# UBC-ECE-Sasha/PIM-compression

Measured on AMD Instinct MI355X. Metric: end-to-end GB/s (compress + decompress) on Silesia-mix; bit-exact ratio parity, higher is better.
Workload: dtype u8; 1 GPU; silesia_mix 8 x 1024 MiB containers in all (BASELINE configs[4]), block_size 32768; containers_this_rank=8, container_bytes=1073741824, block_size=32768, parallelism=whole containers dealt over 1 GPU(s), no collective

## Files before the change

### pim-compression_amd/csrc/snappy_k1_stream.hpp

```cpp
#pragma once

namespace snappy_hip {


#ifdef SNAPPY_PROF
__device__ unsigned long long g_prof[32];
struct StreamProf {
    unsigned long long acc = 0, cnt = 0, last = 0;
};
#define PROF_START() (prof.last = __builtin_readcyclecounter())
#define PROF_LAP(i) do { const unsigned long long now_ = __builtin_readcyclecounter(); if (lane == (i)) { prof.acc += now_ - prof.last; prof.cnt++; } prof.last = now_; } while (0)
#define PROF_WAIT() __builtin_amdgcn_s_waitcnt(0)
#define PROF_FLUSH() do { if (lane < 16) { atomicAdd(&g_prof[lane], prof.acc); atomicAdd(&g_prof[16 + lane], prof.cnt); } } while (0)
#elif defined(SNAPPY_MARK)
struct StreamProf {};
#define PROF_START() asm volatile("; PHASE start")
#define PROF_LAP(i) asm volatile("; PHASE " #i)
#define PROF_WAIT() ((void)0)
#define PROF_FLUSH() ((void)0)
#else
struct StreamProf {};
#define PROF_START() ((void)0)
#define PROF_LAP(i) ((void)0)
#define PROF_WAIT() ((void)0)
#define PROF_FLUSH() ((void)0)
#endif

template <class T, class = void> struct table_gathers_once : std::false_type {};
template <class T> struct table_gathers_once<T, std::void_t<decltype(T::kGathersOnce)>> : std::true_type {};

constexpr uint32_t kStreamRoom = 192;
#ifndef SNAPPY_STREAM_SLOTS_LDS
#define SNAPPY_STREAM_SLOTS_LDS 512
#endif
constexpr uint32_t kStreamSlotsLds = SNAPPY_STREAM_SLOTS_LDS, kStreamSlotsGlobal = 256;
__host__ __device__ constexpr uint32_t stream_scratch_bytes(uint32_t slots) { return 8u * slots; }

struct StreamWindow {
    uint32_t base;
    uint4 a, b;
    uint32_t h0, e0;
};

__device__ __forceinline__ void stream_load_window(StreamWindow& w, const uint8_t* __restrict__ blk, uint32_t base, uint32_t last16,
                                                   uint32_t lane)
{
    w.base = base;
    const uint32_t q = base + lane;
    w.a = ld128(blk + (q < last16 ? q : last16));
    w.b = ld128(blk + (q + 16u < last16 ? q + 16u : last16));
}
__device__ __forceinline__ void stream_hash_window(StreamWindow& w, uint32_t shift)
{
    const uint32_t prod = w.a.x * kHashMul;
    w.h0 = prod >> shift;
    w.e0 = (prod << (32 - shift)) & 0xffff0000u;
}

struct StreamGather {
    uint32_t ent;
    uint4 ka, kb;
    unsigned long long worthm;
};
template <class Table>
__device__ __forceinline__ void stream_issue_gather(StreamGather& g, const Table& table, const StreamWindow& w,
                                                    const uint8_t* __restrict__ blk, uint32_t lane)
{
    const uint32_t mine_l = w.e0 | (w.base + lane);
    g.ent = table.load_lane(w.h0, mine_l);
    const bool worth = !Table::certain_miss(g.ent, mine_l);
    g.worthm = __ballot(worth);
    g.ka = g.kb = make_uint4(0, 0, 0, 0);
    if (worth) {
        const uint8_t* __restrict__ c = blk + (g.ent & 0xffffu);
        g.ka = ld128(c);
        g.kb = ld128(c + 16);
    }
}

#ifdef SNAPPY_EMU
__device__ __forceinline__ uint32_t lds_max_rtn(lds_words_t p, uint32_t v)
{
    const uint32_t old = *p;
    if (v > old) *p = v;
    return old;
}
#else
__device__ __forceinline__ uint32_t lds_max_rtn(lds_words_t p, uint32_t v)
{
    return __hip_atomic_fetch_max((__attribute__((address_space(3))) uint32_t*)p, v, __ATOMIC_RELAXED, __HIP_MEMORY_SCOPE_WAVEFRONT);
}
#endif

struct StreamDup {
    uint32_t j1 = 0;
    uint32_t extj = 0;
    unsigned long long nf = 0;
    unsigned long long hitj = 0;
    unsigned long long deep = 0;
    unsigned long long cx = 0;
};

template <uint32_t kSlots>
__device__ __forceinline__ void stream_analyse(StreamDup& d, const StreamWindow& w, lds_bytes_t scratch, uint32_t lane)
{
    lds_words_t tab = (lds_words_t)scratch;
    const uint32_t sa = w.h0 & (kSlots - 1u);
    const uint32_t sb = kSlots + ((w.h0 >> 5) & (kSlots - 1u));
#ifdef SNAPPY_EMU
    static const bool unordered = getenv("EMU_LDS_UNORDERED") != nullptr;
    uint32_t oa = 0, ob = 0;
    if (unordered) {
        oa = lds_max_rtn(tab + sa, lane + 1u);
        ob = lds_max_rtn(tab + sb, lane + 1u);
    } else {
        for (uint32_t turn = 0; turn < kWave; ++turn) {
            if (lane == turn) {
                oa = lds_max_rtn(tab + sa, lane + 1u);
                ob = lds_max_rtn(tab + sb, lane + 1u);
            }
            __builtin_amdgcn_wave_barrier();
        }
    }
#else
    const uint32_t oa = lds_max_rtn(tab + sa, lane + 1u);
    const uint32_t ob = lds_max_rtn(tab + sb, lane + 1u);
#endif
    __builtin_amdgcn_wave_barrier();
    tab[sa] = 0;
    tab[sb] = 0;
    __builtin_amdgcn_wave_barrier();
    const uint32_t ja = oa - 1u, jb = ob - 1u;
    d = StreamDup();
    if (__ballot((oa && ja >= lane) || (ob && jb >= lane))) {
        STREAM_STAT(7);
        ALIAS_STAT(3);
        d.cx = dup_slot_lanes(scratch, w.h0, lane);
        for (uint32_t i = lane; i < 2u * kSlots; i += kWave) tab[i] = 0;
        __builtin_amdgcn_wave_barrier();
        return;
    }
    const uint32_t ha = (uint32_t)__shfl((int)w.h0, (int)(ja & 63u));
    const uint32_t hb = (uint32_t)__shfl((int)w.h0, (int)(jb & 63u));
    const unsigned long long OA = __ballot(oa != 0), OB = __ballot(ob != 0);
    const unsigned long long MA = OA & __ballot(ha == w.h0), MB = OB & __ballot(hb == w.h0);
    const bool ma = __builtin_amdgcn_inverse_ballot_w64(MA);
    d.j1 = ma ? ja : jb;
    d.nf = MA | MB;
    d.cx = OA & OB & ~d.nf;
    for (unsigned long long m = d.cx; m; m &= m - 1) {
        const uint32_t s = (uint32_t)__builtin_ctzll(m);
        const uint32_t hs = (uint32_t)__builtin_amdgcn_readlane((int)w.h0, (int)s);
        ALIAS_STAT(0);
        if (__ballot(w.h0 == hs) & ((1ull << s) - 1ull)) {
            ALIAS_STAT(2);
        } else {
            ALIAS_STAT(1);
            d.cx &= ~(1ull << s);
        }
    }
    if (d.nf) {
        const uint32_t jl = d.j1 & 63u;
        const uint32_t xj = (uint32_t)__shfl((int)w.a.x, (int)jl);
        const uint32_t e1 = (uint32_t)__shfl((int)w.a.y, (int)jl) ^ w.a.y;
        const uint32_t e2 = (uint32_t)__shfl((int)w.a.z, (int)jl) ^ w.a.z;
        d.hitj = d.nf & __ballot(xj == w.a.x);
        d.extj = min_u32(min_u32(first_bit(e1), first_bit(e2) | 32u), 64u) >> 3;
        const unsigned long long chained = d.nf | d.cx;
        d.deep = d.nf & __ballot(((uint32_t)(chained >> jl) & 1u) != 0);
    }
}

__device__ __forceinline__ void stream_walk(uint32_t advv, uint32_t clv, uint32_t& t, unsigned long long& V, unsigned long long& COV)
{
#ifdef SNAPPY_EMU
    for (;;) {
        const uint32_t l = t & 63u;
        V |= 1ull << l;
        const uint32_t a = (uint32_t)__builtin_amdgcn_readlane((int)advv, (int)l);
        const uint32_t c = (uint32_t)__builtin_amdgcn_readlane((int)clv, (int)l);
        if (c) COV |= ((1ull << c) - 1ull) << l;
        const uint32_t nt = t + a;
        const bool carry = nt < t;
        t = nt;
        if (carry) break;
    }
#else
    uint32_t a, c;
    unsigned long long m;
    asm volatile(
        "1:\n"
        "  s_bitset1_b64 %[V], %[t]\n"
        "  v_readlane_b32 %[a], %[advv], %[t]\n"
        "  v_readlane_b32 %[c], %[clv], %[t]\n"
        "  s_bfm_b64 %[m], %[c], %[t]\n"
        "  s_or_b64 %[COV], %[COV], %[m]\n"
        "  s_add_u32 %[t], %[t], %[a]\n"
        "  s_cbranch_scc1 2f\n"
        "  s_bitset1_b64 %[V], %[t]\n"
        "  v_readlane_b32 %[a], %[advv], %[t]\n"
        "  v_readlane_b32 %[c], %[clv], %[t]\n"
        "  s_bfm_b64 %[m], %[c], %[t]\n"
        "  s_or_b64 %[COV], %[COV], %[m]\n"
        "  s_add_u32 %[t], %[t], %[a]\n"
        "  s_cbranch_scc1 2f\n"
        "  s_bitset1_b64 %[V], %[t]\n"
        "  v_readlane_b32 %[a], %[advv], %[t]\n"
        "  v_readlane_b32 %[c], %[clv], %[t]\n"
        "  s_bfm_b64 %[m], %[c], %[t]\n"
        "  s_or_b64 %[COV], %[COV], %[m]\n"
        "  s_add_u32 %[t], %[t], %[a]\n"
        "  s_cbranch_scc1 2f\n"
        "  s_bitset1_b64 %[V], %[t]\n"
        "  v_readlane_b32 %[a], %[advv], %[t]\n"
        "  v_readlane_b32 %[c], %[clv], %[t]\n"
        "  s_bfm_b64 %[m], %[c], %[t]\n"
        "  s_or_b64 %[COV], %[COV], %[m]\n"
        "  s_add_u32 %[t], %[t], %[a]\n"
        "  s_cbranch_scc0 1b\n"
        "2:\n"
        : [t] "+s"(t), [V] "+s"(V), [COV] "+s"(COV), [a] "=&s"(a), [c] "=&s"(c), [m] "=&s"(m)
        : [advv] "v"(advv), [clv] "v"(clv)
        : "scc");
#endif
}

#ifndef SNAPPY_EMU
__device__ __forceinline__ unsigned long long uni64(unsigned long long v)
{
    return (unsigned long long)uni((uint32_t)v) | ((unsigned long long)uni((uint32_t)(v >> 32)) << 32);
}
#else
__device__ __forceinline__ unsigned long long uni64(unsigned long long v) { return v; }
#endif

__device__ __forceinline__ uint32_t stream_past(uint32_t dist, unsigned long long inter, uint32_t land)
{
    if (land >= kWave || ((inter >> land) & 1ull)) return 0;
    return (uint32_t)__builtin_amdgcn_readlane((int)dist, (int)land);
}

__device__ __forceinline__ bool has_run_of_34(unsigned long long m)
{
    unsigned long long r = m & (m >> 1);
    r &= r >> 2;
    r &= r >> 4;
    r &= r >> 8;
    r &= r >> 16;
    return (r & (m >> 32) & (m >> 33)) != 0;
}

template <class Table>
__device__ __forceinline__ void stream_put(const Table& table, uint32_t x, uint32_t pos, uint32_t shift, uint32_t lane)
{
    const uint32_t prod = x * kHashMul;
    if constexpr (Table::kCollectiveStore)
        table.store_masked(1ull, prod >> shift, pos, lane);
    else
        table.put(prod >> shift, ((prod << (32 - shift)) & 0xffff0000u) | pos, lane);
}
template <class Table>
__device__ __forceinline__ void stream_store(const Table& table, const StreamWindow& w, unsigned long long m, uint32_t lane)
{
    if constexpr (Table::kCollectiveStore) {
        table.store_masked(m, w.h0, w.base + lane, lane);
    } else {
        if (__builtin_amdgcn_inverse_ballot_w64(m)) table.store_lane(w.h0, w.e0 | (w.base + lane));
        __builtin_amdgcn_wave_barrier();
    }
}

__device__ __forceinline__ void stream_emit(uint8_t* __restrict__ dst, const uint8_t* __restrict__ blk, uint32_t& op, uint32_t& next_emit,
                                            uint32_t base, uint32_t x0, uint32_t ent, uint32_t extv, unsigned long long H,
                                            unsigned long long COV, bool by_copy, uint32_t r_out, bool long_copy, uint32_t ip,
                                            uint32_t long_cand, uint32_t long_len, uint32_t lane)
{
    if (H) emit_segment<false>(dst, blk, op, next_emit, base, x0, ent, extv, H, COV, by_copy, r_out, lane);
    if (long_copy) {
        if (ip > next_emit) op = emit_literal_windowed<false>(dst, op, blk, next_emit, ip - next_emit, base, x0, lane);
        op = emit_copy(dst, op, ip - long_cand, long_len, lane);
        next_emit = ip + long_len;
    }
}

struct SoloMate {
    static constexpr bool kAnalysesInPlace = true;
    __device__ __forceinline__ void begin(uint32_t, uint32_t, uint32_t) {}
    __device__ __forceinline__ void drain(uint32_t&, uint32_t&, uint32_t) {}
    template <uint32_t kSlots>
    __device__ __forceinline__ void analysis(StreamDup& d, const StreamWindow& w, lds_bytes_t scratch, uint32_t lane)
    {
        stream_analyse<kSlots>(d, w, scratch, lane);
    }
    __device__ __forceinline__ void emit(uint8_t* __restrict__ dst, const uint8_t* __restrict__ blk, uint32_t& op, uint32_t& next_emit,
                                         uint32_t base, uint32_t x0, uint32_t ent, uint32_t extv, unsigned long long H,
                                         unsigned long long COV, bool by_copy, uint32_t r_out, bool long_copy, uint32_t ip,
                                         uint32_t long_cand, uint32_t long_len, uint32_t lane)
    {
        stream_emit(dst, blk, op, next_emit, base, x0, ent, extv, H, COV, by_copy, r_out, long_copy, ip, long_cand, long_len, lane);
    }
};

template <class Table, uint32_t kSlots, class Mate>
__device__ __forceinline__ void stream_run(const uint8_t* __restrict__ blk, uint32_t avail, uint32_t n, uint32_t shift,
                                           uint8_t* __restrict__ dst, const Table table, uint32_t lane, lds_bytes_t dup_scratch,
                                           ParseState& ps, StreamProf& prof, Mate& mate)
{
    const uint32_t limit = n - kInputMargin;
    const uint32_t last16 = avail - 16u;
    uint32_t ip = ps.ip, skip = ps.skip, op = ps.op, next_emit = ps.next_emit;
    mate.begin(op, next_emit, lane);

    for (;;) {
        StreamWindow cur, nxt;
        stream_load_window(cur, blk, ip & ~63u, last16, lane);
        stream_hash_window(cur, shift);
        StreamGather g;
        stream_issue_gather(g, table, cur, blk, lane);
        __builtin_amdgcn_sched_barrier(0);
        stream_load_window(nxt, blk, cur.base + 64u, last16, lane);
        StreamDup dup;
        mate.template analysis<kSlots>(dup, cur, dup_scratch, lane);
        PROF_LAP(0);
        bool restart = false;

        for (;;) {
            const uint32_t r0 = ip - cur.base;
            const uint32_t b_in = 64u - skip;
            PROF_WAIT();
            PROF_LAP(1);

            unsigned long long hitm = __ballot(g.ka.x == cur.a.x) & g.worthm;
            const uint32_t t1 = min_u32(first_bit(g.ka.y ^ cur.a.y), first_bit(g.ka.z ^ cur.a.z) | 32u);
            const uint32_t t2 = min_u32(first_bit(g.ka.w ^ cur.a.w), first_bit(g.kb.x ^ cur.b.x) | 32u) | 64u;
            const uint32_t t3 = min_u32(first_bit(g.kb.y ^ cur.b.y), first_bit(g.kb.z ^ cur.b.z) | 32u) | 128u;
            uint32_t extv = min_u32(min_u32(t1, t2), min_u32(t3, 192u)) >> 3;
            uint32_t ent = g.ent & 0xffffu;
            const unsigned long long pend = dup.nf & __ballot(dup.j1 >= r0);
            const unsigned long long satm = hitm & __ballot(extv == 24u);
            unsigned long long stopm = pend | dup.cx | satm;
            const unsigned long long above_r0 = ~0ull << r0;
            const unsigned long long inter = hitm | stopm;
            const unsigned long long up = (lane < 63u) ? (inter >> (lane + 1u)) : 0ull;
            const uint32_t dist = up ? (uint32_t)__builtin_ctzll(up) + 1u : 64u - lane;
            const bool stopl = __builtin_amdgcn_inverse_ballot_w64(stopm);
            const bool hitl = __builtin_amdgcn_inverse_ballot_w64(hitm);
            const uint32_t clt = hitl ? 4u + extv : 0u;
            const bool hitjl = __builtin_amdgcn_inverse_ballot_w64(dup.hitj);
            const uint32_t clj = hitjl ? 4u + dup.extj : 0u;
            const uint32_t land_t = lane + clt, land_j = lane + clj;
            const uint32_t dist_t = (uint32_t)__shfl((int)dist, (int)(land_t & 63u));
            const uint32_t dist_j = (uint32_t)__shfl((int)dist, (int)(land_j & 63u));
            const bool plain_t = land_t < 64u && !((inter >> (land_t & 63u)) & 1ull);
            const bool plain_j = land_j < 64u && !((inter >> (land_j & 63u)) & 1ull);
            const uint32_t advt = hitl ? clt + (plain_t ? dist_t : 0u) : dist;
            const uint32_t advj = hitjl ? clj + (plain_j ? dist_j : 0u) : dist;
            const unsigned long long satjm = dup.hitj & __ballot(dup.extj == 8u);
            uint32_t clv = stopl ? 0u : clt;
            uint32_t advv = stopl ? 64u : advt;
            PROF_LAP(2);

            unsigned long long V = 0, COV = 0;
            uint32_t t = r0 - 64u;
            uint32_t r_out = 0;
            bool long_copy = false;
            uint32_t long_cand = 0, long_len = 0;
            for (;;) {
                t = uni(t);
                stream_walk(advv, clv, t, V, COV);
                const uint32_t s = 63u - (uint32_t)__builtin_clzll(V);
                if (!((stopm >> s) & 1ull)) {
                    r_out = t + 64u;
                    break;
                }
                PROF_LAP(3);
                STREAM_STAT(3);
                const unsigned long long bit_s = 1ull << s;
                const unsigned long long below_s = bit_s - 1ull;
                const unsigned long long interior_s = COV & ~(V & hitm & below_s);
                uint32_t how = 0;
                uint32_t j = 0;
                if (pend & bit_s) {
                    j = (uint32_t)__builtin_amdgcn_readlane((int)dup.j1, (int)s);
                    const unsigned long long not_inserted = interior_s & (interior_s >> 1);
                    if (!((not_inserted >> j) & 1ull)) how = 1;
                    else if (dup.deep & bit_s) how = 2;
                }
                if (dup.cx & bit_s) how = 2;
#ifdef SNAPPY_EMU
                if (dup.cx & bit_s) ALIAS_STAT(4);
                else if (!(pend & bit_s)) ALIAS_STAT(8);
                else if (how == 2) ALIAS_STAT(5);
                else if (how == 1) ALIAS_STAT(7);
                else ALIAS_STAT(6);
#endif
                uint32_t adv_s, cl_s, cand_s = 0, sat_s = 24;
                bool hit_s, more_s;
                if (how == 2) {
                    STREAM_STAT(6);
                    const unsigned long long ins = ((above_r0 & below_s & ~interior_s) | (COV & ~(interior_s >> 1))) & below_s;
                    const uint32_t hs = (uint32_t)__builtin_amdgcn_readlane((int)cur.h0, (int)s);
                    const unsigned long long J = __ballot(cur.h0 == hs) & ins;
                    how = 0;
                    if (!J) ALIAS_STAT(9);
                    if (J) {
                        j = 63u - (uint32_t)__builtin_clzll(J);
                        hit_s = (uint32_t)__builtin_amdgcn_readlane((int)cur.a.x, (int)s) == (uint32_t)__builtin_amdgcn_readlane((int)cur.a.x, (int)j);
                        const uint32_t e1 = (uint32_t)__builtin_amdgcn_readlane((int)cur.a.y, (int)s) ^ (uint32_t)__builtin_amdgcn_readlane((int)cur.a.y, (int)j);
                        const uint32_t e2 = (uint32_t)__builtin_amdgcn_readlane((int)cur.a.z, (int)s) ^ (uint32_t)__builtin_amdgcn_readlane((int)cur.a.z, (int)j);
                        const uint32_t ext_s = e1 ? ((uint32_t)__builtin_ctz(e1) >> 3) : (e2 ? 4u + ((uint32_t)__builtin_ctz(e2) >> 3) : 8u);
                        cand_s = cur.base + j;
                        sat_s = 8;
                        more_s = hit_s && ext_s == 8u;
                        cl_s = hit_s ? 4u + ext_s : 0u;
                        adv_s = hit_s ? cl_s : (uint32_t)__builtin_amdgcn_readlane((int)dist, (int)s);
                        if (hit_s && !more_s) adv_s += stream_past(dist, hitm | stopm, s + cl_s);
                        how = 3;
                    }
                }
                if (how == 1) {
                    STREAM_STAT(9);
                    hit_s = (dup.hitj & bit_s) != 0;
                    more_s = (satjm & bit_s) != 0;
                    adv_s = (uint32_t)__builtin_amdgcn_readlane((int)advj, (int)s);
                    cl_s = (uint32_t)__builtin_amdgcn_readlane((int)clj, (int)s);
                    cand_s = cur.base + j;
                    sat_s = 8;
                } else if (how == 0) {
                    STREAM_STAT(10);
                    hit_s = (hitm & bit_s) != 0;
                    more_s = (satm & bit_s) != 0;
                    adv_s = (uint32_t)__builtin_amdgcn_readlane((int)advt, (int)s);
                    cl_s = (uint32_t)__builtin_amdgcn_readlane((int)clt, (int)s);
                }
                if (more_s) {
                    STREAM_STAT(8);
                    if (how == 0) cand_s = (uint32_t)__builtin_amdgcn_readlane((int)ent, (int)s);
                    cl_s = 4u + sat_s + match_extend(blk, cand_s + 4u + sat_s, cur.base + s + 4u + sat_s, n, lane);
                    adv_s = cl_s <= 63u ? cl_s + stream_past(dist, hitm | stopm, s + cl_s) : cl_s;
                    if (cl_s > 63u) {
                        STREAM_STAT(2);
                        V &= ~bit_s;
                        r_out = s;
                        long_copy = true;
                        long_cand = cand_s;
                        long_len = cl_s;
                        break;
                    }
                }
                stopm &= ~bit_s;
                hitm = hit_s ? (hitm | bit_s) : (hitm & ~bit_s);
                if (lane == s) {
                    advv = adv_s;
                    clv = cl_s;
                    if (how != 0) ent = cand_s;
                    if (how != 0 || more_s) extv = cl_s - 4u;
                }
                t = s - 64u;
                PROF_LAP(4);
            }
            PROF_LAP(3);

            const uint32_t r_end = r_out < kWave ? r_out : kWave;
            const unsigned long long range = r_end > r0 ? (above_r0 & lanes_below(r_end)) : 0ull;
            const unsigned long long H = V & hitm & range;
            const unsigned long long interior = COV & ~H;
            const unsigned long long probed = range & ~interior;
            const unsigned long long miss = probed & ~H;
            const uint32_t top = probed ? 63u - (uint32_t)__builtin_clzll(probed) : 0u;
            const bool by_copy = probed && ((H >> top) & 1ull);
            uint32_t skip_out = skip;
            bool widened = false;
            if (probed) {
                const uint32_t tail = by_copy ? 0u : (uint32_t)__builtin_clzll(~(miss << (63u - top)));
                const bool copy_before = (H & ((1ull << top) - 1ull)) != 0;
                const uint32_t allowed = copy_before ? 33u : b_in;
                if ((uint32_t)__builtin_popcountll(miss) > b_in) {
                    const uint32_t lead = (uint32_t)__builtin_ctzll(~(miss >> r0));
                    widened = lead > b_in || has_run_of_34(miss) || tail > allowed;
                }
                skip_out = by_copy ? 31u : 64u - (allowed - tail);
            }
            if (widened) {
                STREAM_STAT(1);
                break;
            }
            STREAM_STAT(0);

            unsigned long long endl = COV & ~(interior >> 1) & range;
            if (by_copy && r_out > kWave) endl &= ~(1ull << 63);
            unsigned long long C = probed | endl;
            if (long_copy) C |= 1ull << r_out;
            {
                const unsigned long long later = dup.nf | dup.cx;
                stream_store(table, cur, C & ~later, lane);
                const unsigned long long second = C & dup.nf & ~dup.deep & ~dup.cx;
                if (second) stream_store(table, cur, second, lane);
                for (unsigned long long dd = C & (dup.deep | dup.cx); dd; dd &= dd - 1) stream_store(table, cur, dd & (~dd + 1), lane);
            }
            ip = cur.base + r_out;
            skip = skip_out;
            PROF_LAP(5);

            const bool go = !long_copy && skip < 64u && cur.base + 64u + kStreamRoom <= limit;
            const StreamWindow old = cur;
            const uint32_t old_ent = ent, old_extv = extv;
            if (go) {
                cur = nxt;
                stream_hash_window(cur, shift);
                if (r_out > kWave) {
                    stream_store(table, cur, 1ull << (r_out - kWave - 1u), lane);
                }
                __builtin_amdgcn_sched_barrier(0);
                stream_load_window(nxt, blk, cur.base + 64u, last16, lane);
                stream_issue_gather(g, table, cur, blk, lane);
                __builtin_amdgcn_sched_barrier(0);
            }
            PROF_LAP(6);

            if (H || long_copy)
                mate.emit(dst, blk, op, next_emit, old.base, old.a.x, old_ent, old_extv, H, COV, by_copy, r_out, long_copy, ip, long_cand,
                          long_len, lane);
            PROF_LAP(7);

            if (long_copy) {
                ip += long_len;
                skip = 31;
                if (ip < limit) {
                    stream_put(table, uld32(blk + ip - 1u), ip - 1u, shift, lane);
                    restart = (ip & ~63u) + kStreamRoom <= limit;
                }
                PROF_LAP(9);
                break;
            }
            if (!go) {
                if (r_out > kWave)
                    stream_put(table, uld32(blk + ip - 1u), ip - 1u, shift, lane);
                break;
            }
            mate.template analysis<kSlots>(dup, cur, dup_scratch, lane);
            PROF_LAP(8);
        }
        if (!restart) break;
    }
    mate.drain(op, next_emit, lane);
    ps.ip = ip;
    ps.skip = skip;
    ps.op = op;
    ps.next_emit = next_emit;
}

template <class Table, uint32_t kSlots, class Mate>
__device__ __forceinline__ void compress_one_block_stream(const uint8_t* __restrict__ base16, uint64_t start, uint64_t in_len,
                                                          uint32_t n, uint8_t* __restrict__ dst, const Table table_in, uint32_t lane,
                                                          uint32_t* __restrict__ block_bytes_out, lds_bytes_t dup_scratch, Mate& mate)
{
    const uint8_t* __restrict__ blk = base16 + start;
    const uint32_t ts = table_entries_for(n);
    const uint32_t shift = (uint32_t)__builtin_clz(ts) + 1;
    const uint32_t e_zero = (n >= kInputMargin) ? (((uld32(blk) * kHashMul) << (32 - shift)) & 0xffff0000u) : 0u;
    const Table table = table_in.with_empty(e_zero);
    if (n >= kInputMargin) table.init(ts, e_zero, lane);
    if (Mate::kAnalysesInPlace)
        for (uint32_t i = lane; i < 2u * kSlots; i += kWave) ((lds_words_t)dup_scratch)[i] = 0;
    __builtin_amdgcn_wave_barrier();
    ParseState ps;
    StreamProf prof;
    PROF_START();
    if (n >= kInputMargin) {
        const uint32_t limit = n - kInputMargin;
        const uint64_t left = in_len - start;
        const uint32_t avail = (left < 0x7fffffffull) ? (uint32_t)left : 0x7fffffffu;
        for (;;) {
            if (ps.skip < 64u && (ps.ip & ~63u) + kStreamRoom <= limit) {
                STREAM_STAT(4);
                PROF_LAP(12);
                stream_run<Table, kSlots, Mate>(blk, avail, n, shift, dst, table, lane, dup_scratch, ps, prof, mate);
                if (ps.ip >= limit) break;
            }
            STREAM_STAT(5);
            const bool over = bulk_run<Table, 64, table_gathers_once<Table>::value>(blk, avail, n, shift, dst, table, lane, dup_scratch, ps,
                                                                                    (ps.ip | 63u) + 1u);
            if (Mate::kAnalysesInPlace)
                for (uint32_t i = lane; i < 2u * kSlots; i += kWave) ((lds_words_t)dup_scratch)[i] = 0;
            __builtin_amdgcn_wave_barrier();
            PROF_LAP(11);
            if (over) break;
        }
    }
    finish_block(blk, n, dst, ps, lane, block_bytes_out);
    PROF_LAP(12);
    PROF_FLUSH();
}

}
```

### pim-compression_amd/csrc/snappy_kernels.hpp

```cpp
#pragma once
#include <hip/hip_runtime.h>
#include <type_traits>
#include <stdint.h>
#ifdef SNAPPY_EMU
#include <stdio.h>
#include <stdlib.h>
#endif

#include "snappy_device_common.hpp"

namespace snappy_hip {

constexpr uint32_t kMaxTableEntries = 16384;
constexpr uint32_t kHashMul = 0x1e35a7bdu;
constexpr uint32_t kInputMargin = 15;

#if defined(__HIP_DEVICE_COMPILE__)
#define SNAPPY_PIN(x) asm volatile("" : "+v"(x))
#else
#define SNAPPY_PIN(x) ((void)0)
#endif

constexpr uint32_t kBlockOk = 0;
constexpr uint32_t kBlockInvalid = 1;
constexpr uint32_t kRangeOutOfBounds = 2;

__device__ __forceinline__ uint32_t table_entries_for(uint32_t n)
{
    uint32_t ts = 256;
    while (ts < kMaxTableEntries && ts < n) ts <<= 1;
    return ts;
}


template <bool kWide = true>
__device__ __forceinline__ uint32_t emit_literal(uint8_t* __restrict__ dst, uint32_t op,
                                                 const uint8_t* __restrict__ src, uint32_t len, uint32_t lane)
{
    const uint32_t n = len - 1;
    uint32_t hdr;
    if (n < 60) {
        hdr = 1;
        if (lane == 0) dst[op] = (uint8_t)(n << 2);
    } else {
        const uint32_t cnt = (n < 256u) ? 1u : ((n < 65536u) ? 2u : 3u);
        hdr = 1 + cnt;
        if (lane < hdr)
            dst[op + lane] = (lane == 0) ? (uint8_t)((59 + cnt) << 2) : (uint8_t)(n >> (8 * (lane - 1)));
    }
    uint8_t* d = dst + op + hdr;
    if (len <= kWave) {
        if (lane < len) d[lane] = src[lane];
    } else if (kWide && len >= 1024u) {
        uint32_t base = 0;
        for (; base + 64u * kWave <= len; base += 64u * kWave) {
            const uint8_t* __restrict__ s = src + (base + 16u * lane);
            uint8_t* __restrict__ t = d + (base + 16u * lane);
            const uint4 v0 = ld128(s), v1 = ld128(s + 16u * kWave), v2 = ld128(s + 32u * kWave), v3 = ld128(s + 48u * kWave);
            st128(t, v0);
            st128(t + 16u * kWave, v1);
            st128(t + 32u * kWave, v2);
            st128(t + 48u * kWave, v3);
        }
        const uint32_t last = len - 16u;
        for (; base < len; base += 16u * kWave) {
            const uint32_t i = base + 16u * lane;
            const uint32_t o = i < last ? i : last;
            st128(d + o, ld128(src + o));
        }
    } else {
        uint32_t i = 4 * lane;
        for (; i + 4 <= len; i += 4 * kWave) st32(d + i, ld32(src + i));
        for (; i < len; ++i) d[i] = src[i];
    }
    return op + hdr + len;
}

__device__ __forceinline__ uint32_t emit_copy_piece(uint8_t* __restrict__ dst, uint32_t op, uint32_t off,
                                                    uint32_t len, uint32_t lane)
{
    if (len < 12 && off < 2048) {
        if (lane < 2)
            dst[op + lane] = (lane == 0) ? (uint8_t)(1 + ((len - 4) << 2) + ((off >> 8) << 5)) : (uint8_t)(off & 0xff);
        return op + 2;
    }
    if (lane < 3)
        dst[op + lane] = (lane == 0) ? (uint8_t)(2 + ((len - 1) << 2))
                                     : ((lane == 1) ? (uint8_t)(off & 0xff) : (uint8_t)(off >> 8));
    return op + 3;
}

__device__ __forceinline__ uint32_t emit_copy(uint8_t* __restrict__ dst, uint32_t op, uint32_t off, uint32_t len,
                                              uint32_t lane)
{
    if (len > 64) {
        const uint32_t n64 = (len >= 68) ? ((len - 68) / 64 + 1) : 0;
        len -= 64 * n64;
        const uint32_t has60 = (len > 64) ? 1u : 0u;
        if (has60) len -= 60;
        const uint32_t nfull = n64 + has60;
        for (uint32_t k = lane; k < nfull; k += kWave) {
            const uint32_t plen = (k < n64) ? 64u : 60u;
            uint8_t* p = dst + op + 3 * k;
            p[0] = (uint8_t)(2 + ((plen - 1) << 2));
            p[1] = (uint8_t)(off & 0xff);
            p[2] = (uint8_t)(off >> 8);
        }
        op += 3 * nfull;
    }
    return emit_copy_piece(dst, op, off, len, lane);
}

__device__ __forceinline__ uint32_t match_extend(const uint8_t* __restrict__ blk, uint32_t a, uint32_t b, uint32_t n,
                                                 uint32_t lane)
{
    uint32_t m = 0;
    for (;;) {
        const uint32_t pb = b + m + 4 * lane;
        const uint32_t pa = a + m + 4 * lane;
        uint32_t eq;
        if (pb + 4 <= n) {
            const uint32_t x = ld32(blk + pa) ^ ld32(blk + pb);
            eq = x ? ((uint32_t)__builtin_ctz(x) >> 3) : 4u;
        } else {
            eq = 0;
            for (uint32_t k = 0; pb + k < n; ++k) {
                if (blk[pa + k] != blk[pb + k]) break;
                ++eq;
            }
        }
        const unsigned long long stop = __ballot(eq != 4);
        if (stop == 0) {
            m += 4 * kWave;
            continue;
        }
        const uint32_t first = (uint32_t)__builtin_ctzll(stop);
        return m + 4 * first + (uint32_t)__builtin_amdgcn_readlane((int)eq, (int)first);
    }
}

struct CursorWindow {
    const uint8_t* __restrict__ blk;
    uint32_t avail;
    uint32_t shift;
    uint32_t base;
    uint32_t x0, h0, e0;
    uint32_t x1;

    __device__ __forceinline__ void rehash()
    {
        const uint32_t prod = x0 * kHashMul;
        h0 = prod >> shift;
        e0 = (prod << (32 - shift)) & 0xffff0000u;
    }

    __device__ __forceinline__ uint32_t load_at(uint32_t pos, uint32_t lane) const
    {
        const uint32_t q = pos + lane;
        const uint32_t last = avail - 4;
        return ld32(blk + ((q < last) ? q : last));
    }
    __device__ __forceinline__ void reset(uint32_t pos, uint32_t lane)
    {
        base = pos & ~63u;
        x0 = load_at(base, lane);
        rehash();
        __builtin_amdgcn_sched_barrier(0);
        x1 = load_at(base + 64, lane);
    }
    __device__ __forceinline__ bool ensure(uint32_t pos, uint32_t lane)
    {
        if (pos < base + 64) return false;
        if (pos < base + 128) {
            base += 64;
            x0 = x1;
            rehash();
            __builtin_amdgcn_sched_barrier(0);
            x1 = load_at(base + 64, lane);
        } else {
            reset(pos, lane);
        }
        return true;
    }
    __device__ __forceinline__ uint32_t bytes_at(uint32_t pos) const
    {
        return (uint32_t)__builtin_amdgcn_readlane((int)x0, (int)(pos - base));
    }
    __device__ __forceinline__ uint32_t hash_at(uint32_t pos) const
    {
        return (uint32_t)__builtin_amdgcn_readlane((int)h0, (int)(pos - base));
    }
    __device__ __forceinline__ uint32_t entry_at(uint32_t pos) const
    {
        return (uint32_t)__builtin_amdgcn_readlane((int)e0, (int)(pos - base)) | pos;
    }
    __device__ __forceinline__ uint32_t bytes_near(uint32_t pos) const
    {
        const uint32_t rel = pos - base;
        if (rel < 64) return (uint32_t)__builtin_amdgcn_readlane((int)x0, (int)rel);
        uint32_t v = x1;
        SNAPPY_PIN(v);
        return (uint32_t)__builtin_amdgcn_readlane((int)v, (int)(rel - 64));
    }
};

#ifdef SNAPPY_EMU
typedef volatile uint8_t* lds_bytes_t;
typedef volatile uint32_t* lds_words_t;
__device__ __forceinline__ void lds_or(lds_words_t p, uint32_t v) { *p = *p | v; }
__device__ __forceinline__ void lds_and(lds_words_t p, uint32_t v) { *p = *p & v; }
#else
typedef volatile __attribute__((address_space(3))) uint8_t* lds_bytes_t;
typedef volatile __attribute__((address_space(3))) uint32_t* lds_words_t;
__device__ __forceinline__ void lds_or(lds_words_t p, uint32_t v)
{
    __hip_atomic_fetch_or((__attribute__((address_space(3))) uint32_t*)p, v, __ATOMIC_RELAXED, __HIP_MEMORY_SCOPE_WAVEFRONT);
}
__device__ __forceinline__ void lds_and(lds_words_t p, uint32_t v)
{
    __hip_atomic_fetch_and((__attribute__((address_space(3))) uint32_t*)p, v, __ATOMIC_RELAXED, __HIP_MEMORY_SCOPE_WAVEFRONT);
}
#endif

#ifdef SNAPPY_EMU
__device__ __forceinline__ uint32_t lds_ld32u(lds_bytes_t p)
{
    uint32_t v;
    __builtin_memcpy(&v, (const void*)p, 4);
    return v;
}
__device__ __forceinline__ void lds_st32u(lds_bytes_t p, uint32_t v) { __builtin_memcpy((void*)p, &v, 4); }
#else
typedef uint32_t __attribute__((aligned(1))) lds_u32_unaligned_t;
__device__ __forceinline__ uint32_t lds_ld32u(lds_bytes_t p)
{
    return *reinterpret_cast<volatile __attribute__((address_space(3))) lds_u32_unaligned_t*>(p);
}
__device__ __forceinline__ void lds_st32u(lds_bytes_t p, uint32_t v)
{
    *reinterpret_cast<volatile __attribute__((address_space(3))) lds_u32_unaligned_t*>(p) = v;
}
#endif

#ifdef SNAPPY_EMU
inline uint32_t g_emu_store_index[16][kWave];
__device__ __forceinline__ void emu_check_distinct_stores(bool stores, uint32_t index, uint32_t lane)
{
    uint32_t* mine = g_emu_store_index[blockIdx.x & 15u];
    mine[lane] = stores ? index : 0xffffffffu;
    __builtin_amdgcn_wave_barrier();
    if (stores)
        for (uint32_t l = 0; l < kWave; ++l)
            if (l != lane && mine[l] == index) {
                fprintf(stderr, "emulator: lanes %u and %u store to table entry %u in one instruction\n", lane, l, index);
                abort();
            }
    __builtin_amdgcn_wave_barrier();
}
#else
__device__ __forceinline__ void emu_check_distinct_stores(bool, uint32_t, uint32_t) {}
#endif

#ifdef SNAPPY_EMU
inline unsigned long long g_stream_stats[16] = {0};
#define STREAM_STAT(i) do { if (lane == 0) ++g_stream_stats[i]; } while (0)
inline unsigned long long g_alias_stats[16] = {0};
#define ALIAS_STAT(i) do { if (lane == 0) ++g_alias_stats[i]; } while (0)
#else
#define STREAM_STAT(i) ((void)0)
#define ALIAS_STAT(i) ((void)0)
#endif

struct FilteredGlobalTable {
    static constexpr bool kCollectiveStore = false;
    uint32_t* __restrict__ t;
    lds_words_t written;
    uint32_t empty;
    __device__ __forceinline__ void init(uint32_t entries, uint32_t, uint32_t lane) const
    {
        for (uint32_t i = lane; i < entries / 32; i += kWave) written[i] = 0;
        __builtin_amdgcn_wave_barrier();
    }
    __device__ __forceinline__ bool is_written(uint32_t h) const { return (written[h >> 5] >> (h & 31u)) & 1u; }
    __device__ __forceinline__ uint32_t exchange(uint32_t h, uint32_t entry, uint32_t lane) const
    {
        uint32_t hv = h;
        SNAPPY_PIN(hv);
        uint32_t old = empty;
        if (is_written(hv)) old = t[hv];
        old = uni(old);
        t[hv] = entry;
        if (lane == 0) lds_or(written + (h >> 5), 1u << (h & 31u));
        __builtin_amdgcn_wave_barrier();
        return old;
    }
    __device__ __forceinline__ void put(uint32_t h, uint32_t entry, uint32_t lane) const
    {
        uint32_t hv = h;
        SNAPPY_PIN(hv);
        t[hv] = entry;
        if (lane == 0) lds_or(written + (h >> 5), 1u << (h & 31u));
        __builtin_amdgcn_wave_barrier();
    }
    __device__ __forceinline__ static bool certain_miss(uint32_t old, uint32_t entry) { return ((old ^ entry) >> 16) != 0; }
    __device__ __forceinline__ uint32_t load_lane(uint32_t h, uint32_t = 0) const { return is_written(h) ? t[h] : empty; }
    __device__ __forceinline__ void store_lane(uint32_t h, uint32_t entry) const
    {
        t[h] = entry;
        lds_or(written + (h >> 5), 1u << (h & 31u));
    }
    __device__ __forceinline__ FilteredGlobalTable with_empty(uint32_t e) const { return FilteredGlobalTable{t, written, e}; }
};

template <uint32_t kSlots>
struct CachedGlobalTable {
    static constexpr bool kCollectiveStore = true;
    uint16_t* __restrict__ t;
    lds_words_t written;
    lds_words_t cache;
    __device__ __forceinline__ void init(uint32_t entries, uint32_t, uint32_t lane) const
    {
        for (uint32_t i = lane; i < entries / 32; i += kWave) written[i] = 0;
        for (uint32_t i = lane; i < kSlots; i += kWave) cache[i] = 0;
        __builtin_amdgcn_wave_barrier();
    }
    __device__ __forceinline__ bool is_written(uint32_t h) const { return (written[h >> 5] >> (h & 31u)) & 1u; }
    __device__ __forceinline__ static bool certain_miss(uint32_t, uint32_t) { return false; }
    __device__ __forceinline__ CachedGlobalTable with_empty(uint32_t) const { return *this; }
    __device__ __forceinline__ uint32_t load_lane(uint32_t h, uint32_t mine) const
    {
        const uint32_t w = cache[h & (kSlots - 1u)];
        const bool wr = is_written(h);
        uint32_t pos = w & 0xffffu;
        if ((w >> 16) != h + 1u) pos = wr ? (uint32_t)t[h] : 0u;
        return (mine & 0xffff0000u) | pos;
    }
    __device__ __forceinline__ void store_masked(unsigned long long m, uint32_t h, uint32_t pos, uint32_t lane) const
    {
        const bool s = __builtin_amdgcn_inverse_ballot_w64(m);
        const uint32_t idx = h & (kSlots - 1u), mine = ((h + 1u) << 16) | (pos & 0xffffu);
        const uint32_t old = cache[idx];
        __builtin_amdgcn_wave_barrier();
        if (s) {
            cache[idx] = mine;
            lds_or(written + (h >> 5), 1u << (h & 31u));
        }
        __builtin_amdgcn_wave_barrier();
        const uint32_t now = cache[idx];
        const bool lost = s && now != mine;
        const bool evicts = s && !lost && old != 0u && (old >> 16) != h + 1u;
        if (evicts) t[(old >> 16) - 1u] = (uint16_t)old;
        emu_check_distinct_stores(evicts, (old >> 16) - 1u, lane);
        __builtin_amdgcn_wave_barrier();
        if (__ballot(lost)) {
            if (lost) t[h] = (uint16_t)pos;
            emu_check_distinct_stores(lost, h, lane);
        }
        __builtin_amdgcn_wave_barrier();
    }
};

struct LdsTable {
    static constexpr bool kCollectiveStore = false;
    uint16_t* t;
    __device__ __forceinline__ void init(uint32_t entries, uint32_t, uint32_t lane) const
    {
        uint4* q = reinterpret_cast<uint4*>(t);
        for (uint32_t i = lane; i < entries / 8; i += kWave) q[i] = make_uint4(0, 0, 0, 0);
    }
    __device__ __forceinline__ uint32_t exchange(uint32_t h, uint32_t entry, uint32_t lane) const
    {
        const uint32_t old = uni((uint32_t)t[h]);
        if (lane == 0) t[h] = (uint16_t)entry;
        __builtin_amdgcn_wave_barrier();
        return old;
    }
    __device__ __forceinline__ void put(uint32_t h, uint32_t entry, uint32_t lane) const
    {
        if (lane == 0) t[h] = (uint16_t)entry;
        __builtin_amdgcn_wave_barrier();
    }
    __device__ __forceinline__ static bool certain_miss(uint32_t, uint32_t) { return false; }
    __device__ __forceinline__ uint32_t load_lane(uint32_t h, uint32_t = 0) const { return t[h]; }
    __device__ __forceinline__ void store_lane(uint32_t h, uint32_t entry) const { t[h] = (uint16_t)entry; }
    __device__ __forceinline__ LdsTable with_empty(uint32_t) const { return *this; }
};


__device__ __forceinline__ uint32_t emit_copy_packed(uint8_t* __restrict__ dst, uint32_t op, uint32_t off, uint32_t len,
                                                     uint32_t lane)
{
    if (len > 64) return emit_copy(dst, op, off, len, lane);
    uint32_t word, bytes;
    if (len < 12 && off < 2048) {
        word = (1 + ((len - 4) << 2) + ((off >> 8) << 5)) | ((off & 0xff) << 8);
        bytes = 2;
    } else {
        word = (2 + ((len - 1) << 2)) | (off << 8);
        bytes = 3;
    }
    if (lane == 0) st32(dst + op, word);
    return op + bytes;
}

template <bool kWide = true>
__device__ __forceinline__ uint32_t emit_literal_windowed(uint8_t* __restrict__ dst, uint32_t op,
                                                          const uint8_t* __restrict__ blk, uint32_t from, uint32_t len,
                                                          uint32_t win_base, uint32_t win_x0, uint32_t lane)
{
    if (from < win_base || from + len > win_base + kWave) return emit_literal<kWide>(dst, op, blk + from, len, lane);
    const uint32_t n = len - 1;
    uint32_t hdr;
    if (n < 60) {
        hdr = 1;
        if (lane == 0) dst[op] = (uint8_t)(n << 2);
    } else {
        hdr = 2;
        if (lane == 0) {
            dst[op] = (uint8_t)(60 << 2);
            dst[op + 1] = (uint8_t)n;
        }
    }
    const uint32_t rel = from - win_base;
    if (lane >= rel && lane < rel + len) dst[op + hdr + lane - rel] = (uint8_t)win_x0;
    return op + hdr + len;
}

__constant__ uint32_t kRecip16[64] = {
        0, 65537, 32769, 21846, 16385, 13108, 10923,  9363,  8193,  7282,  6554,  5958,  5462,  5042,  4682,  4370,
     4097,  3856,  3641,  3450,  3277,  3121,  2979,  2850,  2731,  2622,  2521,  2428,  2341,  2260,  2185,  2115,
     2049,  1986,  1928,  1873,  1821,  1772,  1725,  1681,  1639,  1599,  1561,  1525,  1490,  1457,  1425,  1395,
     1366,  1338,  1311,  1286,  1261,  1237,  1214,  1192,  1171,  1150,  1130,  1111,  1093,  1075,  1058,  1041};

constexpr uint32_t kDupSlots = 1024;

__device__ __forceinline__ uint32_t first_bit(uint32_t x) { return (uint32_t)__builtin_ffs((int)x) - 1u; }
__device__ __forceinline__ uint32_t min_u32(uint32_t a, uint32_t b) { return a < b ? a : b; }

__device__ __forceinline__ uint32_t ctz64_or(unsigned long long x, uint32_t if_zero)
{
    return x ? (uint32_t)__builtin_ctzll(x) : if_zero;
}
__device__ __forceinline__ unsigned long long lane_range(uint32_t lo, uint32_t cnt)
{
    return (~0ull >> (64u - cnt)) << lo;
}

__device__ __forceinline__ unsigned long long dup_slot_lanes(lds_bytes_t scratch, uint32_t h, uint32_t lane)
{
    const uint32_t sa = h & (kDupSlots / 2 - 1);
    const uint32_t sb = kDupSlots / 2 + ((h >> 5) & (kDupSlots / 2 - 1));
    scratch[sa] = (uint8_t)lane;
    scratch[sb] = (uint8_t)lane;
    __builtin_amdgcn_wave_barrier();
    const uint32_t wa = scratch[sa];
    const uint32_t wb = scratch[sb];
    __builtin_amdgcn_wave_barrier();
    if (wa != lane) scratch[sa] = 0xff;
    if (wb != lane) scratch[sb] = 0xff;
    __builtin_amdgcn_wave_barrier();
    const uint32_t ma = scratch[sa];
    const uint32_t mb = scratch[sb];
    __builtin_amdgcn_wave_barrier();
    return __ballot(ma == 0xff && mb == 0xff);
}
__device__ __forceinline__ unsigned long long dup_slot_lanes_among(lds_bytes_t scratch, uint32_t h, bool on, uint32_t lane)
{
    const uint32_t sa = h & (kDupSlots / 2 - 1);
    const uint32_t sb = kDupSlots / 2 + ((h >> 5) & (kDupSlots / 2 - 1));
    if (on) {
        scratch[sa] = (uint8_t)lane;
        scratch[sb] = (uint8_t)lane;
    }
    __builtin_amdgcn_wave_barrier();
    uint32_t wa = lane, wb = lane;
    if (on) {
        wa = scratch[sa];
        wb = scratch[sb];
    }
    __builtin_amdgcn_wave_barrier();
    if (wa != lane) scratch[sa] = 0xff;
    if (wb != lane) scratch[sb] = 0xff;
    __builtin_amdgcn_wave_barrier();
    uint32_t ma = 0, mb = 0;
    if (on) {
        ma = scratch[sa];
        mb = scratch[sb];
    }
    __builtin_amdgcn_wave_barrier();
    return __ballot(ma == 0xff && mb == 0xff);
}

template <class Table>
__device__ __forceinline__ uint32_t strided_scan_batch(const Table& table, const uint8_t* __restrict__ blk, uint32_t shift,
                                                       uint32_t limit, uint32_t ip, uint32_t skip, lds_bytes_t dup_scratch,
                                                       uint32_t lane, uint32_t& ip_out, bool& again)
{
    const uint32_t stride0 = skip >> 5;
    const uint32_t c0 = 32u - (skip & 31u);
    const uint32_t over0 = lane > c0 ? lane - c0 : 0u;
    const uint32_t over1 = lane > c0 + 32u ? lane - c0 - 32u : 0u;
    const uint32_t pk = ip + lane * stride0 + over0 + over1;
    const uint32_t stride_k = (skip + lane) >> 5;
    const bool live = pk + stride_k <= limit;
    const unsigned long long livem = __ballot(live);
    const uint32_t x = ld32(blk + (live ? pk : ip));
    const uint32_t prod = x * kHashMul;
    const uint32_t h = prod >> shift;
    const uint32_t mine = ((prod << (32 - shift)) & 0xffff0000u) | pk;
    uint32_t ent = 0;
    if (live) ent = table.load_lane(h, mine);
    const unsigned long long dupm = dup_slot_lanes_among(dup_scratch, h, live, lane);
    const bool worth = live && !Table::certain_miss(ent, mine);
    uint32_t k0 = 0;
    if (worth) k0 = ld32(blk + (ent & 0xffffu));
    const unsigned long long hitm = __ballot(worth) & __ballot(k0 == x);
    unsigned long long stops = hitm | dupm | ~livem;
    uint32_t m;
    again = true;
    STREAM_STAT(11);
    for (;;) {
        m = ctz64_or(stops, kWave);
        if (m == kWave) {
            STREAM_STAT(15);
            break;
        }
        if (!((livem >> m) & 1ull)) {
            STREAM_STAT(14);
            break;
        }
        if ((dupm >> m) & 1ull) {
            const uint32_t hm = (uint32_t)__builtin_amdgcn_readlane((int)h, (int)m);
            if (m && (__ballot(h == hm) & livem & lane_range(0, m))) {
                STREAM_STAT(13);
                break;
            }
        }
        if ((hitm >> m) & 1ull) {
            STREAM_STAT(12);
            again = false;
            break;
        }
        stops &= ~(1ull << m);
    }
    ip_out = m < kWave ? (uint32_t)__builtin_amdgcn_readlane((int)pk, (int)m)
                       : (uint32_t)__builtin_amdgcn_readlane((int)pk, 63) + ((skip + 63u) >> 5);
    if (m) {
        const unsigned long long cm = lane_range(0, m);
        if constexpr (Table::kCollectiveStore) {
            table.store_masked(cm, h, pk, lane);
        } else {
            const bool s = __builtin_amdgcn_inverse_ballot_w64(cm);
            if (s) table.store_lane(h, mine);
            emu_check_distinct_stores(s, h, lane);
            __builtin_amdgcn_wave_barrier();
        }
    }
    return m;
}

template <class Table, uint32_t kChunk>
struct MaskedWindowState {
    uint32_t ent = 0;
    uint32_t extv = 0;
    unsigned long long hit = 0;
    unsigned long long dup = 0;
    unsigned long long longm = 0;
    unsigned long long deepm = 0;
    unsigned long long inserted = 0;
    uint32_t xa = 0, xb = 0;
    uint32_t cov_end = 0;
    bool dup_valid = false;

// ... 1380 lines not shown
```

Before: 65.67 GB/s.

## Resolve simple pending stops inside the scalar stream walk instead of outer loop

Extends the inline-asm stream walk so that, when it lands on a stop lane whose pending dedup choice is simple (not deep/saturated), it decides between the original and alternate candidate in scalar registers and keeps walking. This avoids returning to the heavier vector-level outer loop iteration for each such stop. Packs adv/cl for both choices into one pickv register, records alternate picks in a PJ mask applied after the loop, and adds stats counters. Risks semantic divergence from the outer-loop path and more SGPR pressure.

```diff
diff --git a/pim-compression_amd/csrc/snappy_k1_stream.hpp b/pim-compression_amd/csrc/snappy_k1_stream.hpp
--- a/pim-compression_amd/csrc/snappy_k1_stream.hpp
+++ b/pim-compression_amd/csrc/snappy_k1_stream.hpp
@@ -10,18 +10,21 @@
 };
 #define PROF_START() (prof.last = __builtin_readcyclecounter())
 #define PROF_LAP(i) do { const unsigned long long now_ = __builtin_readcyclecounter(); if (lane == (i)) { prof.acc += now_ - prof.last; prof.cnt++; } prof.last = now_; } while (0)
+#define PROF_COUNT(i, k) do { if (lane == (i)) prof.cnt += (k); } while (0)
 #define PROF_WAIT() __builtin_amdgcn_s_waitcnt(0)
 #define PROF_FLUSH() do { if (lane < 16) { atomicAdd(&g_prof[lane], prof.acc); atomicAdd(&g_prof[16 + lane], prof.cnt); } } while (0)
 #elif defined(SNAPPY_MARK)
 struct StreamProf {};
 #define PROF_START() asm volatile("; PHASE start")
 #define PROF_LAP(i) asm volatile("; PHASE " #i)
+#define PROF_COUNT(i, k) ((void)0)
 #define PROF_WAIT() ((void)0)
 #define PROF_FLUSH() ((void)0)
 #else
 struct StreamProf {};
 #define PROF_START() ((void)0)
 #define PROF_LAP(i) ((void)0)
+#define PROF_COUNT(i, k) ((void)0)
 #define PROF_WAIT() ((void)0)
 #define PROF_FLUSH() ((void)0)
 #endif
@@ -171,23 +174,78 @@
     }
 }
 
-__device__ __forceinline__ void stream_walk(uint32_t advv, uint32_t clv, uint32_t& t, unsigned long long& V, unsigned long long& COV)
+__device__ __forceinline__ void stream_walk(uint32_t advv, uint32_t clv, uint32_t pickv, uint32_t j1, unsigned long long pend,
+                                            unsigned long long deep, unsigned long long satm, unsigned long long satjm,
+                                            unsigned long long hitj, uint32_t& t, unsigned long long& V, unsigned long long& COV,
+                                            unsigned long long& hitm, unsigned long long& stopm, unsigned long long& PJ,
+                                            [[maybe_unused]] uint32_t lane)
 {
 #ifdef SNAPPY_EMU
     for (;;) {
-        const uint32_t l = t & 63u;
-        V |= 1ull << l;
-        const uint32_t a = (uint32_t)__builtin_amdgcn_readlane((int)advv, (int)l);
-        const uint32_t c = (uint32_t)__builtin_amdgcn_readlane((int)clv, (int)l);
-        if (c) COV |= ((1ull << c) - 1ull) << l;
-        const uint32_t nt = t + a;
-        const bool carry = nt < t;
-        t = nt;
-        if (carry) break;
+        uint32_t s;
+        for (;;) {
+            s = t & 63u;
+            V |= 1ull << s;
+            const uint32_t a = (uint32_t)__builtin_amdgcn_readlane((int)advv, (int)s);
+            const uint32_t c = (uint32_t)__builtin_amdgcn_readlane((int)clv, (int)s);
+            if (c) COV |= ((1ull << c) - 1ull) << s;
+            const uint32_t nt = t + a;
+            const bool carry = nt < t;
+            t = nt;
+            if (carry) break;
+        }
+        const unsigned long long bit_s = 1ull << s;
+        if (!(stopm & bit_s)) return;
+        if (!(pend & bit_s)) {
+            PICK_STAT(4);
+            return;
+        }
+        const uint32_t j = (uint32_t)__builtin_amdgcn_readlane((int)j1, (int)s) & 63u;
+        const uint32_t w = (uint32_t)__builtin_amdgcn_readlane((int)pickv, (int)s);
+        const unsigned long long interior_s = COV & ~(V & hitm & (bit_s - 1ull));
+        const unsigned long long not_inserted = interior_s & (interior_s >> 1);
+        uint32_t a, c;
+        if ((not_inserted >> j) & 1ull) {
+            if (deep & bit_s) {
+                PICK_STAT(5);
+                return;
+            }
+            if (satm & bit_s) {
+                PICK_STAT(6);
+                return;
+            }
+            a = w & 0xffu;
+            c = (w >> 8) & 0xffu;
+            PICK_STAT(0);
+            ALIAS_STAT(6);
+            STREAM_STAT(10);
+        } else {
+            if (satjm & bit_s) {
+                PICK_STAT(7);
+                return;
+            }
+            PJ |= bit_s;
+            hitm = (hitm & ~bit_s) | (hitj & bit_s);
+            a = (w >> 16) & 0xffu;
+            c = w >> 24;
+            PICK_STAT(1);
+            ALIAS_STAT(7);
+            STREAM_STAT(9);
+        }
+        STREAM_STAT(3);
+        stopm &= ~bit_s;
+        if (c) COV |= ((1ull << c) - 1ull) << s;
+        const uint32_t t0 = s - 64u;
+        t = t0 + a;
+        if (t < t0) {
+            PICK_STAT(2);
+            return;
+        }
     }
 #else
-    uint32_t a, c;
-    unsigned long long m;
+    uint32_t a, c, s, j, w;
+    unsigned long long m, q;
+    const unsigned long long slow_t = deep | satm;
     asm volatile(
         "1:\n"
         "  s_bitset1_b64 %[V], %[t]\n"
@@ -219,8 +277,49 @@
         "  s_add_u32 %[t], %[t], %[a]\n"
         "  s_cbranch_scc0 1b\n"
         "2:\n"
-        : [t] "+s"(t), [V] "+s"(V), [COV] "+s"(COV), [a] "=&s"(a), [c] "=&s"(c), [m] "=&s"(m)
-        : [advv] "v"(advv), [clv] "v"(clv)
+        "  s_sub_u32 %[s], %[t], %[a]\n"
+        "  s_bitcmp1_b64 %[stopm], %[s]\n"
+        "  s_cbranch_scc0 9f\n"
+        "  ; PICK begin\n"
+        "  s_bitcmp1_b64 %[pend], %[s]\n"
+        "  s_cbranch_scc0 9f\n"
+        "  v_readlane_b32 %[j], %[j1], %[s]\n"
+        "  v_readlane_b32 %[w], %[pickv], %[s]\n"
+        "  s_and_b64 %[m], %[V], %[hitm]\n"
+        "  s_bfm_b64 %[q], %[s], 0\n"
+        "  s_and_b64 %[m], %[m], %[q]\n"
+        "  s_andn2_b64 %[q], %[COV], %[m]\n"
+        "  s_lshr_b64 %[m], %[q], 1\n"
+        "  s_and_b64 %[q], %[q], %[m]\n"
+        "  s_bitcmp1_b64 %[q], %[j]\n"
+        "  s_cbranch_scc0 5f\n"
+        "  s_bitcmp1_b64 %[slow_t], %[s]\n"
+        "  s_cbranch_scc1 9f\n"
+        "  s_and_b32 %[a], %[w], 0xff\n"
+        "  s_bfe_u32 %[c], %[w], 0x80008\n"
+        "  s_branch 6f\n"
+        "5:\n"
+        "  s_bitcmp1_b64 %[satjm], %[s]\n"
+        "  s_cbranch_scc1 9f\n"
+        "  s_bitset1_b64 %[PJ], %[s]\n"
+        "  s_bitset0_b64 %[hitm], %[s]\n"
+        "  s_lshl_b64 %[m], 1, %[s]\n"
+        "  s_and_b64 %[m], %[m], %[hitj]\n"
+        "  s_or_b64 %[hitm], %[hitm], %[m]\n"
+        "  s_bfe_u32 %[a], %[w], 0x80010\n"
+        "  s_lshr_b32 %[c], %[w], 24\n"
+        "6:\n"
+        "  s_bitset0_b64 %[stopm], %[s]\n"
+        "  s_bfm_b64 %[m], %[c], %[s]\n"
+        "  s_or_b64 %[COV], %[COV], %[m]\n"
+        "  s_add_u32 %[t], %[s], %[a]\n"
+        "  s_cbranch_scc0 1b\n"
+        "  ; PICK end\n"
+        "9:\n"
+        : [t] "+s"(t), [V] "+s"(V), [COV] "+s"(COV), [hitm] "+s"(hitm), [stopm] "+s"(stopm), [PJ] "+s"(PJ), [a] "=&s"(a),
+          [c] "=&s"(c), [s] "=&s"(s), [j] "=&s"(j), [w] "=&s"(w), [m] "=&s"(m), [q] "=&s"(q)
+        : [advv] "v"(advv), [clv] "v"(clv), [pickv] "v"(pickv), [j1] "v"(j1), [pend] "s"(pend), [slow_t] "s"(slow_t),
+          [satjm] "s"(satjm), [hitj] "s"(hitj)
         : "scc");
 #endif
 }
@@ -358,16 +457,24 @@
             const unsigned long long satjm = dup.hitj & __ballot(dup.extj == 8u);
             uint32_t clv = stopl ? 0u : clt;
             uint32_t advv = stopl ? 64u : advt;
+            const uint32_t pickv = advt | (clt << 8) | (advj << 16) | (clj << 24);
             PROF_LAP(2);
 
-            unsigned long long V = 0, COV = 0;
+            unsigned long long V = 0, COV = 0, PJ = 0;
+            [[maybe_unused]] uint32_t picks = 0;
             uint32_t t = r0 - 64u;
             uint32_t r_out = 0;
             bool long_copy = false;
             uint32_t long_cand = 0, long_len = 0;
             for (;;) {
                 t = uni(t);
-                stream_walk(advv, clv, t, V, COV);
+#if defined(SNAPPY_EMU) || defined(SNAPPY_PROF)
+                const unsigned long long stop_in = stopm;
+#endif
+                stream_walk(advv, clv, pickv, dup.j1, pend, dup.deep, satm, satjm, dup.hitj, t, V, COV, hitm, stopm, PJ, lane);
+#if defined(SNAPPY_EMU) || defined(SNAPPY_PROF)
+                picks += (uint32_t)__builtin_popcountll(stop_in & ~stopm);
+#endif
                 const uint32_t s = 63u - (uint32_t)__builtin_clzll(V);
                 if (!((stopm >> s) & 1ull)) {
                     r_out = t + 64u;
@@ -422,16 +529,18 @@
                     STREAM_STAT(9);
                     hit_s = (dup.hitj & bit_s) != 0;
                     more_s = (satjm & bit_s) != 0;
-                    adv_s = (uint32_t)__builtin_amdgcn_readlane((int)advj, (int)s);
-                    cl_s = (uint32_t)__builtin_amdgcn_readlane((int)clj, (int)s);
+                    const uint32_t w_s = (uint32_t)__builtin_amdgcn_readlane((int)pickv, (int)s);
+                    adv_s = (w_s >> 16) & 0xffu;
+                    cl_s = w_s >> 24;
                     cand_s = cur.base + j;
                     sat_s = 8;
                 } else if (how == 0) {
                     STREAM_STAT(10);
                     hit_s = (hitm & bit_s) != 0;
                     more_s = (satm & bit_s) != 0;
-                    adv_s = (uint32_t)__builtin_amdgcn_readlane((int)advt, (int)s);
-                    cl_s = (uint32_t)__builtin_amdgcn_readlane((int)clt, (int)s);
+                    const uint32_t w_s = (uint32_t)__builtin_amdgcn_readlane((int)pickv, (int)s);
+                    adv_s = w_s & 0xffu;
+                    cl_s = (w_s >> 8) & 0xffu;
                 }
                 if (more_s) {
                     STREAM_STAT(8);
@@ -460,6 +569,15 @@
                 PROF_LAP(4);
             }
             PROF_LAP(3);
+            PROF_COUNT(10, picks);
+#ifdef SNAPPY_EMU
+            if (picks >= 2u) PICK_STAT(3);
+#endif
+            if (PJ) {
+                const bool pj = __builtin_amdgcn_inverse_ballot_w64(PJ);
+                ent = pj ? cur.base + dup.j1 : ent;
+                extv = pj ? (pickv >> 24) - 4u : extv;
+            }
 
             const uint32_t r_end = r_out < kWave ? r_out : kWave;
             const unsigned long long range = r_end > r0 ? (above_r0 & lanes_below(r_end)) : 0ull;
diff --git a/pim-compression_amd/csrc/snappy_kernels.hpp b/pim-compression_amd/csrc/snappy_kernels.hpp
--- a/pim-compression_amd/csrc/snappy_kernels.hpp
+++ b/pim-compression_amd/csrc/snappy_kernels.hpp
@@ -266,9 +266,12 @@
 #define STREAM_STAT(i) do { if (lane == 0) ++g_stream_stats[i]; } while (0)
 inline unsigned long long g_alias_stats[16] = {0};
 #define ALIAS_STAT(i) do { if (lane == 0) ++g_alias_stats[i]; } while (0)
+inline unsigned long long g_pick_stats[16] = {0};
+#define PICK_STAT(i) do { if (lane == 0) ++g_pick_stats[i]; } while (0)
 #else
 #define STREAM_STAT(i) ((void)0)
 #define ALIAS_STAT(i) ((void)0)
+#define PICK_STAT(i) ((void)0)
 #endif
 
 struct FilteredGlobalTable {
```

Result: no change. 66.21 GB/s (median of 6 runs) (+0.8%).
